# TalShor/SciLMM

Hardware: AMD Instinct MI355X
Metric: REML factorize+solve nnz(L)/s (simulated pedigree, fp64) (higher is better)
Workload: dtype f64

## Files before the change

scilmm_amd/csrc/dev.h:

```cpp
#pragma once
#include <hip/hip_runtime.h>

#include <algorithm>
#include <cstdlib>
#include <optional>
#include <string>
#include <type_traits>
#include <vector>

#include "../../include/scilmm_hip.h"
#include "plan_types.h"
#include "handles.h"

namespace scilmm {

struct Tuning {
  int reserve_cus = 0;
  int side_streams = 2;
  bool no_mfma = false;
  bool trsm_lite = true;
  std::optional<bool> dense;
  std::optional<bool> outside;
  bool outside_merge = true;
  std::optional<int> outside_chunks;
  bool outside_prio = false;
  std::optional<double> cell_limit;
  bool no_lookahead = false;
  int look_depth = 2;
  bool host_cells = false;
  bool no_splitk = false;
  int64_t target_items = 1024;
  int64_t min_item = 24;
  int64_t max_item = 96;
  std::optional<int64_t> dense_items;
  int64_t dense_fill = 256;
  std::optional<bool> dense_taper;
  std::optional<int> dist_group;
  bool dist_nosplit = false;
  int chain_cap = 2048;
  int chain_wide = 12;
  bool no_chain = false;
  int64_t push_slice = 512;
  bool shadow = true;
  int chain_wide_t = 160;
  int chain_full_t = 768;
  bool chain_pipe = true;
  int chain_stagger = 0;
  bool sinv_generic = false;
  bool sinv_reverse = false;
  int sinv_cc_tiles = 2;
};

inline Tuning read_tuning() {
  Tuning t;
  const char* gate = getenv("SCILMM_TUNING");
  if (!(gate && gate[0] == '1')) return t;
  auto env = [](const char* name) { return getenv(name); };
  auto is1 = [&](const char* name) { const char* e = env(name); return e && e[0] == '1'; };
  auto not0 = [&](const char* name) { const char* e = env(name); return !(e && e[0] == '0'); };
  const char* e;
  if ((e = env("SCILMM_RESERVE_CUS"))) t.reserve_cus = atoi(e);
  if ((e = env("SCILMM_SIDE_STREAMS"))) t.side_streams = atoi(e);
  t.no_mfma = is1("SCILMM_NO_MFMA");
  t.trsm_lite = not0("SCILMM_TRSM_LITE");
  if ((e = env("SCILMM_DENSE"))) t.dense = e[0] != '0';
  if ((e = env("SCILMM_OUTSIDE"))) t.outside = e[0] != '0';
  t.outside_merge = not0("SCILMM_OUTSIDE_MERGE");
  if ((e = env("SCILMM_OUTSIDE_CHUNKS"))) t.outside_chunks = atoi(e);
  t.outside_prio = is1("SCILMM_OUTSIDE_PRIO");
  if ((e = env("SCILMM_CELL_LIMIT"))) t.cell_limit = atof(e);
  t.no_lookahead = is1("SCILMM_NO_LOOKAHEAD");
  if ((e = env("SCILMM_LOOK_DEPTH"))) t.look_depth = std::max(1, atoi(e));
  t.host_cells = is1("SCILMM_HOST_CELLS");
  t.no_splitk = is1("SCILMM_NO_SPLITK");
  if ((e = env("SCILMM_TARGET_ITEMS"))) t.target_items = atoll(e);
  if ((e = env("SCILMM_MIN_ITEM"))) t.min_item = atoll(e);
  if ((e = env("SCILMM_MAX_ITEM"))) t.max_item = atoll(e);
  if ((e = env("SCILMM_DENSE_ITEMS"))) t.dense_items = atoll(e);
  if ((e = env("SCILMM_DENSE_FILL"))) t.dense_fill = atoll(e);
  if ((e = env("SCILMM_DENSE_TAPER"))) t.dense_taper = e[0] == '1';
  if ((e = env("SCILMM_DIST_GROUP"))) t.dist_group = atoi(e);
  t.dist_nosplit = is1("SCILMM_DIST_NOSPLIT");
  if ((e = env("SCILMM_CHAIN_CAP"))) t.chain_cap = atoi(e);
  if ((e = env("SCILMM_CHAIN_WIDE"))) t.chain_wide = atoi(e);
  t.no_chain = is1("SCILMM_NO_CHAIN");
  if ((e = env("SCILMM_PUSH_SLICE"))) t.push_slice = atoll(e);
  t.shadow = not0("SCILMM_SHADOW");
  if ((e = env("SCILMM_CHAIN_WIDE_T"))) t.chain_wide_t = atoi(e);
  if ((e = env("SCILMM_CHAIN_FULL_T"))) t.chain_full_t = atoi(e);
  t.chain_pipe = not0("SCILMM_CHAIN_PIPE");
  if ((e = env("SCILMM_CHAIN_STAGGER"))) t.chain_stagger = std::max(0, atoi(e));
  t.sinv_generic = is1("SCILMM_SINV_GENERIC");
  t.sinv_reverse = is1("SCILMM_SINV_REVERSE");
  if ((e = env("SCILMM_SINV_CC_TILES"))) t.sinv_cc_tiles = std::max(1, atoi(e));
  return t;
}

inline bool verbose() { return getenv("SCILMM_VERBOSE") != nullptr; }

struct Dev {
  int device = 0;
  hipStream_t stream = nullptr;
  Tuning tune;
  int prio_lo = 0, prio_hi = 0;
  DevSym v{};
  std::vector<void*> allocs;
  int32_t* d_level_tiles = nullptr;
// ... 293 lines not shown
```

scilmm_amd/csrc/kernels.hip.h:

```cpp
#pragma once
#include <hip/hip_runtime.h>
#ifndef SCILMM_UPD_WAVES
#define SCILMM_UPD_WAVES 2
#endif
#include <stdint.h>
#include <type_traits>

#include "plan_types.h"

namespace scilmm {

typedef double d4 __attribute__((ext_vector_type(4)));

constexpr int NJB = NB / 16;
constexpr int KCS = 16;
constexpr int LDA = TM + 16;
constexpr int LDB = NB + 16;
constexpr int LDP = 34;

__device__ __forceinline__ d4 mfma_f64(double a, double b, d4 c) {
  return __builtin_amdgcn_mfma_f64_16x16x4f64(a, b, c, 0, 0, 0);
}

__global__ void k_assemble(int64_t nnz, const int64_t* __restrict__ dst, ValPtrs vp, double* __restrict__ L) {
// ... 291 lines not shown
  if (wk.slot < 0) {
    double* P = L + S.sn_loff[s];
#pragma unroll
    for (int jb = 0; jb < NJB; ++jb)
#pragma unroll
      for (int r = 0; r < 4; ++r) {
        const int j = 16 * jb + lr + 4 * r;
        const int i = 16 * wv + li;
        if (i < nrow && j < w) P[(int64_t)j * m + R0 + i] -= acc[jb][r];
      }
  } else {
    double* Q = scratch + (int64_t)wk.slot * (TM * NB);
#pragma unroll
    for (int jb = 0; jb < NJB; ++jb)
#pragma unroll
      for (int r = 0; r < 4; ++r) {
        const int j = 16 * jb + lr + 4 * r;
        const int i = 16 * wv + li;
        Q[j * TM + i] = acc[jb][r];
      }
  }
}


#ifndef SCILMM_DENSE_ABL
#define SCILMM_DENSE_ABL 0
#endif
#ifndef SCILMM_DENSE_VEC
#define SCILMM_DENSE_VEC 1
#endif
constexpr int DTR = 2 * TM;
constexpr int KBA = 64;
constexpr int LDA2 = DTR + 16;

#ifdef SCILMM_DENSE_CLK
__device__ unsigned long long g_dense_clk[2];
#endif

__device__ __forceinline__ int64_t uniform_i64(int64_t x) {
  const uint64_t v = (uint64_t)x;
  const uint32_t lo = __builtin_amdgcn_readfirstlane((uint32_t)v), hi = __builtin_amdgcn_readfirstlane((uint32_t)(v >> 32));
  return (int64_t)(((uint64_t)hi << 32) | lo);
}
__device__ __forceinline__ double ld_off(const double* base, uint32_t voff8) {
  return *(const double*)((const char*)base + voff8);
}
__device__ __forceinline__ int uniform_int(int v) { return __builtin_amdgcn_readfirstlane(v); }
typedef __attribute__((address_space(3))) void* lds_vptr;
typedef const __attribute__((address_space(1))) void* gl_vptr;

#ifndef SCILMM_DENSE_B_SG
#define SCILMM_DENSE_B_SG 1
#endif
__global__ __launch_bounds__(512, 1) void k_dense_b(DevSym S, int32_t dense_first, const DenseWork* __restrict__ work,
                                                    double* __restrict__ L, double* __restrict__ scratch,
                                                    const double* __restrict__ zeros) {
  static_assert(NB == 128 && DTR == 256, "k_dense_b: 8 waves x 32 rows, one B k-row per DMA instruction");
  extern __shared__ __attribute__((aligned(16))) double smem[];
  const int tid = threadIdx.x, lane = tid & 63, wv = __builtin_amdgcn_readfirstlane(tid >> 6);
  const int li = lane & 15, lk = lane >> 4;
  const DenseWork wk = work[blockIdx.x];
  const int32_t j = wk.front;
  const int32_t c0j = S.sn_start[j], wj = S.sn_start[j + 1] - c0j;
  const int32_t mj = S.n - c0j;
  const int32_t R0 = wk.ti0 * TM;
  const int32_t nrow = min(wk.ntiles * TM, mj - R0);
  const int32_t ia = 32 * wv + li, ib_ = ia + 16;
  const int32_t ra0 = R0 + (ia < nrow ? ia : 0);
  const int32_t ra1 = R0 + (ib_ < nrow ? ib_ : 0);
  const int32_t b_off = 2 * lane < wj ? 2 * lane : 0;
  const double* zsrc = zeros + 2 * lane;
  struct Chunk { const double* Pd; int32_t md; int kc; uint32_t v0, v1; };
  int32_t kd = wk.k0, kk0 = 0;
  int32_t d_wd = 0, d_md = 0;
  const double* d_P0 = nullptr;
  auto next_chunk = [&]() {
    if (kk0 == 0) {
      const int32_t d = dense_first + kd;
      const int32_t c0d = S.sn_start[d];
      d_wd = __builtin_amdgcn_readfirstlane(S.sn_start[d + 1] - c0d);
      d_md = __builtin_amdgcn_readfirstlane(S.n - c0d);
      d_P0 = L + uniform_i64(S.sn_loff[d] + (c0j - c0d));
    }
    Chunk c;
    c.md = d_md;
    c.Pd = d_P0 + (int64_t)kk0 * d_md;
    c.kc = min(KBA, d_wd - kk0);
    c.v0 = (uint32_t)(lk * c.md + ra0) * 8u;
    c.v1 = (uint32_t)(lk * c.md + ra1) * 8u;
    kk0 += KBA;
    if (kk0 >= d_wd) { kk0 = 0; ++kd; }
    return c;
  };
  auto issue_B = [&](const Chunk& c, int b) {
    double* Bs = smem + b * KBA * LDB;
    if (c.kc == KBA) {
      const double* p = c.Pd + (int64_t)wv * c.md + b_off;
      const int64_t step = 8 * (int64_t)c.md;
#pragma unroll
      for (int i = 0; i < KBA / 8; ++i)
        __builtin_amdgcn_global_load_lds((gl_vptr)(p + i * step), (lds_vptr)(Bs + (wv + 8 * i) * LDB), 16, 0, 0);
      return;
    }
#pragma unroll
    for (int i = 0; i < KBA / 8; ++i) {
      const int kr = wv + 8 * i;
      __builtin_amdgcn_global_load_lds((gl_vptr)(kr < c.kc ? c.Pd + (int64_t)kr * c.md + b_off : zsrc), (lds_vptr)(Bs + kr * LDB), 16, 0, 0);
    }
  };
  auto load_A = [&](const Chunk& c, int s, double (&ra)[4][2]) {
    const int klast = (c.kc - 1) & ~3;
#pragma unroll
    for (int q = 0; q < 4; ++q) {
      const double* sp = c.Pd + (int64_t)min(16 * s + 4 * q, klast) * c.md;
      ra[q][0] = ld_off(sp, c.v0);
      ra[q][1] = ld_off(sp, c.v1);
    }
  };
  d4 acc16[NJB][2];
#pragma unroll
  for (int a = 0; a < NJB; ++a) { acc16[a][0] = (d4){0.0, 0.0, 0.0, 0.0}; acc16[a][1] = (d4){0.0, 0.0, 0.0, 0.0}; }
  if (wk.k0 >= wk.k1) return;
  double rA[2][4][2];
  double bf[2][NJB];
  auto ldB = [&](const double* Bc, int k4, double (&b)[NJB]) {
#pragma unroll
    for (int jb = 0; jb < NJB; ++jb) b[jb] = Bc[(k4 + lk) * LDB + 16 * jb + li];
  };
  auto mma = [&](const double (&b)[NJB], double a0, double a1) {
#pragma unroll
    for (int jb = 0; jb < NJB; ++jb) {
      acc16[jb][0] = mfma_f64(b[jb], a0, acc16[jb][0]);
      acc16[jb][1] = mfma_f64(b[jb], a1, acc16[jb][1]);
    }
  };
  Chunk cur = next_chunk();
  issue_B(cur, 0);
  load_A(cur, 0, rA[0]);
  bool more = kd < wk.k1;
  Chunk nxt = cur;
  if (more) {
    nxt = next_chunk();
    issue_B(nxt, 1);
  }
  asm volatile("s_waitcnt vmcnt(0)" ::: "memory");
  __syncthreads();
  int buf = 0;
  ldB(smem, 0, bf[0]);
  while (true) {
    const double* Bc = smem + buf * KBA * LDB;
    const double* Bn = smem + (buf ^ 1) * KBA * LDB;
    bool more2 = false;
    Chunk nn = nxt;
#pragma unroll
    for (int t = 0; t < 16; ++t) {
      const int s = t >> 2, q = t & 3;
      if (q == 0) {
        if (s < 3) load_A(cur, s + 1, rA[(s + 1) & 1]);
        else if (more) load_A(nxt, 0, rA[0]);
      }
      if (t < 15) {
        ldB(Bc, 4 * (t + 1), bf[(t + 1) & 1]);
      } else if (more) {
        asm volatile("s_waitcnt vmcnt(0) lgkmcnt(0)" ::: "memory");
        __builtin_amdgcn_s_barrier();
        ldB(Bn, 0, bf[0]);
        more2 = kd < wk.k1;
        if (more2) {
          nn = next_chunk();
          issue_B(nn, buf);
        }
      }
      mma(bf[t & 1], rA[s & 1][q][0], rA[s & 1][q][1]);
#if SCILMM_DENSE_B_SG
      if (t < 15) {
#pragma unroll
        for (int g = 0; g < 4; ++g) {
          __builtin_amdgcn_sched_group_barrier(0x100, 1, 0);
          __builtin_amdgcn_sched_group_barrier(0x008, 4, 0);
        }
      }
#endif
      __builtin_amdgcn_sched_barrier(0);
    }
    if (!more) break;
    cur = nxt;
    nxt = nn;
    more = more2;
    buf ^= 1;
  }
  double* P = L + S.sn_loff[j];
#pragma unroll
  for (int jb = 0; jb < NJB; ++jb)
#pragma unroll
    for (int ib = 0; ib < 2; ++ib)
#pragma unroll
      for (int r = 0; r < 4; ++r) {
        const int i = ib == 0 ? ia : ib_, jc = 16 * jb + lk + 4 * r;
        const double v = acc16[jb][ib][r];
        const int h = i >> 7;
        const int32_t slot = h ? wk.slot1 : wk.slot0;
        if (slot < 0) {
          if (i < nrow && jc < wj) P[(int64_t)jc * mj + R0 + i] -= v;
        } else if (h < wk.ntiles) {
          scratch[(int64_t)slot * (TM * NB) + jc * TM + (i & (TM - 1))] = v;
        }
      }
}

typedef float f4 __attribute__((ext_vector_type(4)));
constexpr int LDA2F = DTR + 16;
constexpr int LDBF = NB + 16;

__global__ __launch_bounds__(512, 1) void k_dense32(DevSym S, int32_t dense_first, const DenseWork* __restrict__ work,
                                                    double* __restrict__ L, double* __restrict__ scratch) {
  extern __shared__ __attribute__((aligned(16))) double smem[];
  float* Abuf = (float*)smem;
  float* Bbuf = Abuf + 2 * KC * LDA2F;
  const int tid = threadIdx.x, lane = tid & 63, wv = tid >> 6;
  const DenseWork wk = work[blockIdx.x];
  const int32_t j = wk.front;
  const int32_t c0j = S.sn_start[j], wj = S.sn_start[j + 1] - c0j;
  const int32_t mj = S.n - c0j;
  const int32_t R0 = wk.ti0 * TM;
  const int32_t nrow = min(wk.ntiles * TM, mj - R0);
  typedef double d2 __attribute__((ext_vector_type(2)));
  typedef float f2 __attribute__((ext_vector_type(2)));
  constexpr int NPA = KC / 4, NPB = KC / 8;
  const int pa = tid & (DTR / 2 - 1), ka = tid >> 7;
  const int pb = tid & (NB / 2 - 1), kb = tid >> 6;
  const int ra_row = 2 * pa < nrow ? 2 * pa : 0, rb_col = 2 * pb < wj ? 2 * pb : 0;
  d2 ra[NPA], rb[NPB];
  int32_t kd = wk.k0, kk0 = 0;
  int kc_ld = 0;
  auto load_chunk = [&]() {
    const int32_t d = dense_first + kd;
    const int32_t c0d = S.sn_start[d], wd = S.sn_start[d + 1] - c0d;
    const int64_t md = S.n - c0d;
    const double* Pd = L + S.sn_loff[d] + (int64_t)kk0 * md + (c0j - c0d);
    kc_ld = min(KC, wd - kk0);
#pragma unroll
    for (int i = 0; i < NPA; ++i) __builtin_memcpy(&ra[i], Pd + (int64_t)min(ka + 4 * i, kc_ld - 1) * md + R0 + ra_row, 16);
#pragma unroll
    for (int i = 0; i < NPB; ++i) __builtin_memcpy(&rb[i], Pd + (int64_t)min(kb + 8 * i, kc_ld - 1) * md + rb_col, 16);
    kk0 += KC;
    if (kk0 >= wd) { kk0 = 0; ++kd; }
  };
  auto store_chunk = [&](int b) {
    float* As = Abuf + b * KC * LDA2F;
    float* Bs = Bbuf + b * KC * LDBF;
#pragma unroll
    for (int i = 0; i < NPA; ++i) {
      const bool on = ka + 4 * i < kc_ld;
      *(f2*)&As[(ka + 4 * i) * LDA2F + 2 * pa] = (f2){on ? (float)ra[i][0] : 0.0f, on ? (float)ra[i][1] : 0.0f};
    }
#pragma unroll
    for (int i = 0; i < NPB; ++i) {
      const bool on = kb + 8 * i < kc_ld;
      *(f2*)&Bs[(kb + 8 * i) * LDBF + 2 * pb] = (f2){on ? (float)rb[i][0] : 0.0f, on ? (float)rb[i][1] : 0.0f};
    }
  };
  d4 acc[NJB][2];
#pragma unroll
  for (int a = 0; a < NJB; ++a) { acc[a][0] = (d4){0.0, 0.0, 0.0, 0.0}; acc[a][1] = (d4){0.0, 0.0, 0.0, 0.0}; }
  const int li = lane & 15, lk = lane >> 4;
  if (wk.k0 >= wk.k1) return;
  load_chunk();
  int kc_cur = kc_ld;
  store_chunk(0);
  __syncthreads();
  int buf = 0;
  while (true) {
    const bool more = kd < wk.k1;
    if (more) load_chunk();
    const float* Ac = Abuf + buf * KC * LDA2F;
    const float* Bc = Bbuf + buf * KC * LDBF;
    const int kc4 = (kc_cur + 3) & ~3;
    f4 c32[NJB][2];
#pragma unroll
    for (int a = 0; a < NJB; ++a) { c32[a][0] = (f4){0.f, 0.f, 0.f, 0.f}; c32[a][1] = (f4){0.f, 0.f, 0.f, 0.f}; }
#pragma unroll 2
    for (int k4 = 0; k4 < kc4; k4 += 4) {
      const float a0 = Ac[(k4 + lk) * LDA2F + 32 * wv + li], a1 = Ac[(k4 + lk) * LDA2F + 32 * wv + 16 + li];
      float b[NJB];
#pragma unroll
      for (int jb = 0; jb < NJB; ++jb) b[jb] = Bc[(k4 + lk) * LDBF + 16 * jb + li];
#pragma unroll
      for (int jb = 0; jb < NJB; ++jb) {
        c32[jb][0] = __builtin_amdgcn_mfma_f32_16x16x4f32(b[jb], a0, c32[jb][0], 0, 0, 0);
        c32[jb][1] = __builtin_amdgcn_mfma_f32_16x16x4f32(b[jb], a1, c32[jb][1], 0, 0, 0);
      }
    }
#pragma unroll
    for (int jb = 0; jb < NJB; ++jb)
#pragma unroll
      for (int ib = 0; ib < 2; ++ib)
#pragma unroll
        for (int r = 0; r < 4; ++r) acc[jb][ib][r] += (double)c32[jb][ib][r];
    if (!more) break;
    store_chunk(buf ^ 1);
    kc_cur = kc_ld;
    __syncthreads();
    buf ^= 1;
  }
  double* P = L + S.sn_loff[j];
#pragma unroll
  for (int jb = 0; jb < NJB; ++jb)
#pragma unroll
    for (int ib = 0; ib < 2; ++ib)
#pragma unroll
      for (int r = 0; r < 4; ++r) {
        const int i = 32 * wv + 16 * ib + li, jc = 16 * jb + 4 * lk + r;
        const int h = i >> 7;
        const int32_t slot = h ? wk.slot1 : wk.slot0;
        if (slot < 0) {
          if (i < nrow && jc < wj) P[(int64_t)jc * mj + R0 + i] -= acc[jb][ib][r];
        } else if (h < wk.ntiles) {
          scratch[(int64_t)slot * (TM * NB) + jc * TM + (i & (TM - 1))] = acc[jb][ib][r];
        }
      }
}

__global__ __launch_bounds__(256) void k_shadow(const double* __restrict__ src, float* __restrict__ dst, int64_t cnt) {
  for (int64_t i = (int64_t)blockIdx.x * 256 + threadIdx.x; i < cnt; i += (int64_t)gridDim.x * 256) dst[i] = (float)src[i];
}

#ifndef SCILMM_DENSE_H_FOLD
#define SCILMM_DENSE_H_FOLD 4
#endif
#ifndef SCILMM_DENSE_H_WGS
#define SCILMM_DENSE_H_WGS 4
#endif
constexpr int DH_MAXD = 256;
constexpr size_t dense_h_lds = sizeof(float) * 2 * KBA * LDBF + sizeof(int32_t) * (DH_MAXD + 2) + sizeof(int64_t) * DH_MAXD;

__global__ __launch_bounds__(512, SCILMM_DENSE_H_WGS) void k_dense_h(DevSym S, int32_t dense_first, const DenseWork* __restrict__ work,
                                                    double* __restrict__ L, const float* __restrict__ L32, int64_t base32,
                                                    double* __restrict__ scratch, const float* __restrict__ zeros32) {
  static_assert(NB == 128 && TM == 128, "k_dense_h: 4 x 2 waves of 32 rows x 64 columns");
  extern __shared__ __attribute__((aligned(16))) double smem[];
  float* Bimg = (float*)smem;
  int32_t* t_c0 = (int32_t*)(Bimg + 2 * KBA * LDBF);
  int64_t* t_lo = (int64_t*)(t_c0 + DH_MAXD + 2);
  typedef float f2 __attribute__((ext_vector_type(2)));
  constexpr int NJH = NJB / 2;
  const int tid = threadIdx.x, lane = tid & 63, wv = __builtin_amdgcn_readfirstlane(tid >> 6);
  const int rg = wv >> 1, ch = wv & 1;
  const int li = lane & 15, lk = lane >> 4;
  const DenseWork wk = work[blockIdx.x >> 1];
  const int th = blockIdx.x & 1;
  if (th >= wk.ntiles || wk.k0 >= wk.k1) return;
  const int32_t j = wk.front;
  const int32_t c0j = S.sn_start[j], wj = S.sn_start[j + 1] - c0j;
  const int32_t mj = S.n - c0j;
  const int32_t R0 = (wk.ti0 + th) * TM;
  const int32_t nrow = min(TM, mj - R0);
  const int32_t slot = th ? wk.slot1 : wk.slot0;
  const int32_t ndesc = min(wk.k1 - wk.k0, DH_MAXD);
  for (int i = tid; i <= ndesc; i += 512) t_c0[i] = S.sn_start[dense_first + wk.k0 + i];
  for (int i = tid; i < ndesc; i += 512) t_lo[i] = S.sn_loff[dense_first + wk.k0 + i];
  const int32_t ia = 32 * rg + 2 * li;
  const int32_t ra = R0 + (ia < nrow ? ia : 0);
  const int32_t bcol0 = lane < wj ? lane : 0, bcol1 = 64 + lane < wj ? 64 + lane : 0;
  __syncthreads();
  struct Chunk { const float* Pd; int32_t md; int kc; };
  int32_t kd = wk.k0, kk0 = 0;
  auto next_chunk = [&]() {
    const int32_t e = kd - wk.k0, d = dense_first + kd;
    const bool tab = e < DH_MAXD;
    const int32_t c0d = __builtin_amdgcn_readfirstlane(tab ? t_c0[e] : S.sn_start[d]);
    const int32_t wd = __builtin_amdgcn_readfirstlane(tab ? t_c0[e + 1] : S.sn_start[d + 1]) - c0d;
    Chunk c;
    c.md = S.n - c0d;
    c.Pd = L32 + (uniform_i64(tab ? t_lo[e] : S.sn_loff[d]) - base32 + (int64_t)kk0 * c.md + (c0j - c0d));
    c.kc = min(KBA, wd - kk0);
    kk0 += KBA;
    if (kk0 >= wd) { kk0 = 0; ++kd; }
    return c;
  };
  auto issue_B = [&](const Chunk& c, int b) {
    float* Bs = Bimg + b * KBA * LDBF;
#pragma unroll
    for (int i = 0; i < KBA / 8; ++i) {
      const int kr = wv + 8 * i;
      const float* row = c.Pd + (int64_t)kr * c.md;
      const bool on = kr < c.kc;
      __builtin_amdgcn_global_load_lds((gl_vptr)(on ? row + bcol0 : zeros32 + lane), (lds_vptr)(Bs + kr * LDBF), 4, 0, 0);
      __builtin_amdgcn_global_load_lds((gl_vptr)(on ? row + bcol1 : zeros32 + lane), (lds_vptr)(Bs + kr * LDBF + 64), 4, 0, 0);
    }
  };
  auto load_A = [&](const Chunk& c, int s, f2 (&a)[4]) {
    const int klast = (c.kc - 1) & ~3;
    const uint32_t v = (uint32_t)(lk * c.md + ra) * 4u;
#pragma unroll
    for (int q = 0; q < 4; ++q) {
      const float* sp = c.Pd + (int64_t)min(16 * s + 4 * q, klast) * c.md;
      a[q] = *(const f2*)((const char*)sp + v);
    }
  };
  d4 acc[NJH][2];
  f4 c32[NJH][2];
#pragma unroll
  for (int a = 0; a < NJH; ++a) {
    acc[a][0] = (d4){0.0, 0.0, 0.0, 0.0}; acc[a][1] = (d4){0.0, 0.0, 0.0, 0.0};
// ... 2568 lines not shown
```

scilmm_amd/csrc/launch.hip.h:

```cpp
#pragma once

namespace {

int set_attrs(scilmm_symbolic* sym, Dev* D) {
  if (D->attrs_set) return SCILMM_OK;
  const int big = 150 * 1024;
  HIPCHK(hipFuncSetAttribute((const void*)k_potrf, hipFuncAttributeMaxDynamicSharedMemorySize, big));
  HIPCHK(hipFuncSetAttribute((const void*)k_fwd<true, 0, true>, hipFuncAttributeMaxDynamicSharedMemorySize, big));
  HIPCHK(hipFuncSetAttribute((const void*)k_fwd<true, 0, false>, hipFuncAttributeMaxDynamicSharedMemorySize, big));
  HIPCHK(hipFuncSetAttribute((const void*)k_fwd<true, 1, true>, hipFuncAttributeMaxDynamicSharedMemorySize, big));
  HIPCHK(hipFuncSetAttribute((const void*)k_fwd<false, 0, true>, hipFuncAttributeMaxDynamicSharedMemorySize, big));
  HIPCHK(hipFuncSetAttribute((const void*)k_fwd<false, 0, false>, hipFuncAttributeMaxDynamicSharedMemorySize, big));
  HIPCHK(hipFuncSetAttribute((const void*)k_fwd<false, 1, true>, hipFuncAttributeMaxDynamicSharedMemorySize, big));
  HIPCHK(hipFuncSetAttribute((const void*)k_dense32, hipFuncAttributeMaxDynamicSharedMemorySize, big));
  HIPCHK(hipFuncSetAttribute((const void*)k_dense_h, hipFuncAttributeMaxDynamicSharedMemorySize, big));
  HIPCHK(hipFuncSetAttribute((const void*)k_dense_b, hipFuncAttributeMaxDynamicSharedMemorySize, big));
  HIPCHK(hipFuncSetAttribute((const void*)k_update2<true>, hipFuncAttributeMaxDynamicSharedMemorySize, big));
  HIPCHK(hipFuncSetAttribute((const void*)k_update2<false>, hipFuncAttributeMaxDynamicSharedMemorySize, big));
  D->attrs_set = true;
  return SCILMM_OK;
}

inline int64_t max_groups(unsigned threads) { return (int64_t)(((uint64_t)1 << 32) / threads) - 1; }

struct FactorLaunch {
  Dev* const D;
  scilmm_factor* const fac;
  int64_t launches = 0;

  void update(hipStream_t stream, const UpdWork* work, int64_t cnt, double* scratch_half) {
#ifdef SCILMM_DIAG
    if (D->ablate == 4) return;
#endif
    const size_t sm_upd = sizeof(double) * (size_t)(2 * KC * LDA + 2 * KC * LDB) + sizeof(int32_t) * TM;
    const auto k = D->use_mfma ? k_update2<true> : k_update2<false>;
    for (int64_t o = 0; o < cnt; o += max_groups(UPD_THREADS)) {
      const unsigned c = (unsigned)std::min<int64_t>(cnt - o, max_groups(UPD_THREADS));
      hipLaunchKernelGGL(k, dim3(c), dim3(UPD_THREADS), sm_upd, stream, D->v, work + o, D->d_combos, fac->L, scratch_half);
      launches++;
    }
  }

  void dense(hipStream_t stream, const DenseWork* dw, int64_t cnt, double* scratch_half) {
    const int32_t dense_first = fac->sym->S->dense_first;
    for (int64_t o = 0; o < cnt; o += max_groups(1024)) {
      const unsigned c = (unsigned)std::min<int64_t>(cnt - o, max_groups(1024));
      if (D->front_bits == 32 && fac->L32)
        hipLaunchKernelGGL(k_dense_h, dim3(2 * c), dim3(512), dense_h_lds, stream, D->v, dense_first, dw + o, fac->L, (const float*)fac->L32,
                           fac->base32, scratch_half, (const float*)D->d_zeros);
      else if (D->front_bits == 32)
        hipLaunchKernelGGL(k_dense32, dim3(c), dim3(512), sizeof(float) * (size_t)(2 * KC * LDA2F + 2 * KC * LDBF), stream, D->v,
                           dense_first, dw + o, fac->L, scratch_half);
      else
        hipLaunchKernelGGL(k_dense_b, dim3(c), dim3(512), sizeof(double) * (size_t)(2 * KBA * LDB), stream, D->v, dense_first, dw + o,
                           fac->L, scratch_half, (const double*)D->d_zeros);
      launches++;
    }
  }

  void reduce(hipStream_t stream, const int32_t* tiles, int64_t cnt, const int32_t* pslot, const int32_t* pnseg, const double* slabs) {
    const int64_t per = max_groups(128) / (NB / 4);
    for (int64_t o = 0; o < cnt; o += per) {
      const int64_t c = std::min(cnt - o, per);
      hipLaunchKernelGGL(k_reduce, dim3((unsigned)((NB / 4) * c)), dim3(128), 0, stream, D->v, tiles + o, pslot, pnseg, slabs, fac->L);
      launches++;
    }
  }

  int cells(hipStream_t stream, int which, int32_t l) {
    const Dev::CellSet& CS = D->cellset[which];
    const int64_t u0 = CS.level_ptr[l], u1 = CS.level_ptr[l + 1];
    if (u1 <= u0) return SCILMM_OK;
#ifdef SCILMM_DIAG
    if (D->ablate == 5) return SCILMM_OK;
#endif
    const int64_t nshort = CS.level_short[l], nlong = (u1 - u0) - nshort;
    const int64_t nblk = (nshort + 255) / 256 + (nlong + 3) / 4;
    if (nblk > max_groups(256)) {
      fac->sym->err = "cell plan: one level has more target cells than a dispatch can hold";
      return SCILMM_ERR_ARG;
    }
    hipLaunchKernelGGL(k_sparse_cells, dim3((unsigned)nblk), dim3(256), 0, stream, u0, nshort, u1 - u0, (const int64_t*)CS.dst,
                       (const int64_t*)CS.grp, (const int64_t*)CS.srct, (const int64_t*)CS.srcq, (const int32_t*)CS.md,
                       (const int32_t*)CS.wd, fac->L);
    launches++;
    return SCILMM_OK;
  }

  void trsm(hipStream_t stream, const int32_t* tiles, int64_t cnt, const double* slabs) {
    const bool lite = D->use_mfma && D->trsm_lite;
    const auto k = lite ? k_trsm_lite : D->use_mfma ? k_trsm<true> : k_trsm<false>;
    const int64_t per = lite ? max_groups(256) / 4 : max_groups(256);
    for (int64_t o = 0; o < cnt; o += per) {
      const int64_t c = std::min(cnt - o, per);
      hipLaunchKernelGGL(k, dim3((unsigned)(lite ? 4 * c : c)), dim3(256), 0, stream, D->v, tiles + o, fac->L, fac->invD, D->d_tile_pslot,
                         D->d_tile_pnseg, slabs);
      launches++;
    }
  }

  void outside(hipStream_t stream, const OutsideWork* work, int64_t cnt) {
    auto k = D->use_mfma ? k_outside<true> : k_outside<false>;
#ifdef SCILMM_DIAG
    if (D->ablate == 6) k = k_outside<true, 1>;
    if (D->ablate == 7) k = k_outside<true, 2>;
#endif
    for (int64_t o = 0; o < cnt; o += max_groups(256)) {
      const unsigned c = (unsigned)std::min<int64_t>(max_groups(256), cnt - o);
// ... 112 lines not shown
```

scilmm_amd/csrc/plan.hip:

```cpp
#include <hip/hip_runtime.h>

#include <algorithm>
#include <atomic>
#include <chrono>
#include <functional>
#include <thread>
#include <cmath>
#include <cstdio>
#include <cstdlib>
#include <cstring>
#include <string>
#include <vector>

#include "dev.h"
#include "cellplan.hip.h"
#include "host_threads.h"

namespace scilmm {

void dev_free(void* p) {
  Dev* D = (Dev*)p;
  if (!D) return;
  for (void* a : D->allocs) (void)hipFree(a);
  for (double* v : D->vals)
// ... 942 lines not shown
  int st;
  size_t split = 0;
  int64_t ngroups_total = 0;
  if (pb.gpu_cells) {
    int64_t potential = 0;
    std::vector<const std::vector<CellCombo>*> ccparts;
    for (auto& pv : cellparts) {
      ccparts.push_back(&pv);
      for (const CellCombo& q : pv) potential += (int64_t)q.nt * q.nq;
    }
    if (potential >= ((int64_t)1 << 31)) {
      sym->err = "cell plan: more than 2^31 cells (raise SCILMM_CELL_LIMIT granularity or set SCILMM_HOST_CELLS=1)";
      return SCILMM_ERR_ARG;
    }
    int64_t n_early_groups = 0;
    if ((st = build_cells_device(sym, D, ccparts, std::max(S.nlevels, 1), &ngroups_total, &n_early_groups)) != SCILMM_OK) return st;
    split = (size_t)n_early_groups;
    std::vector<std::vector<CellCombo>>().swap(cellparts);
  } else {
    if ((st = build_cells_host(sym, D, pb, &split, &ngroups_total)) != SCILMM_OK) return st;
  }
  {
    if (pb.verbose)
      fprintf(stderr, "[scilmm plan] dense combos %lld, cell-path combos %lld, cells %lld (early %lld) in %lld target groups\n",
              (long long)D->n_dense_combos, (long long)D->n_sparse_combos, (long long)D->n_cells, (long long)split,
              (long long)ngroups_total);
    std::vector<Cell>().swap(cells);
  }
  return SCILMM_OK;
}

struct WorkCut {
  const Symbolic& S;
  Dev* const D;
  const PlanBuild& pb;
  const std::vector<int64_t>&dptr, &dmid;
  std::vector<int32_t> pslot, pnseg, pslot_e, pnseg_e, red_tiles, red_tiles_e;
  std::vector<UpdWork> work, work_early;
  std::vector<DenseWork> dwork_e, dwork_l;
  int64_t max_slots = 0;
  const bool lookahead = !D->tune.no_lookahead;
  const int32_t depth = D->look_depth;
  const bool allow_split = !D->tune.no_splitk;
  const int64_t target_items = D->tune.target_items, min_item = D->tune.min_item, max_item = std::max<int64_t>(min_item, D->tune.max_item);
  const int64_t dense_fill = D->tune.dense_fill;
  const int32_t tail_w = tail_width(S);
  const int64_t dense_items = std::max<int64_t>(64, D->tune.dense_items.value_or(tail_w < 24576 ? 128 : tail_w < 32768 ? 512 : 1024));
  std::vector<std::vector<int32_t>> tail_src;
  std::vector<int32_t> tail_col_front;
  const bool dist = distributed_tail(D, S);
  const int32_t Wg = D->dist_Wg;
  std::vector<std::vector<uint8_t>> own_pair_on;
  int64_t dense_pairs_all = 0, dense_pairs_kept = 0, dense_tiles_all = 0, dense_tiles_kept = 0;

  WorkCut(const Symbolic& S_, Dev* D_, const PlanBuild& pb_) : S(S_), D(D_), pb(pb_), dptr(pb_.dptr), dmid(pb_.dmid) {
    const int64_t ntiles = (int64_t)S.tile_front.size();
    pslot.assign((size_t)std::max<int64_t>(ntiles, 1), 0);
    pnseg.assign(pslot.size(), 0);
    pslot_e.assign(pslot.size(), 0);
    pnseg_e.assign(pslot.size(), 0);
    D->red_ptr_e.assign(S.nlevels + 1, 0);
    D->dwork_e_ptr.assign(S.nlevels + 1, 0);
    D->dwork_l_ptr.assign(S.nlevels + 1, 0);
    D->dwork_l_mid.assign((size_t)std::max(S.nlevels, 1), 0);
    D->work_ptr.assign(S.nlevels + 1, 0);
    D->early_ptr.assign(S.nlevels + 1, 0);
    D->red_ptr.assign(S.nlevels + 1, 0);
    if (D->dense_on && !S.tail_blk_ptr.empty()) {
      const int32_t nT = S.nsuper - S.dense_first;
      tail_src.resize((size_t)nT);
      for (int32_t d = 0; d < nT; ++d)
        for (int64_t e = S.tail_blk_ptr[d]; e < S.tail_blk_ptr[d + 1]; ++e) tail_src[(size_t)S.tail_blk[e]].push_back(d);
    }
    if (!tail_src.empty()) {
      const int32_t c0t = S.sn_start[S.dense_first];
      tail_col_front.resize((size_t)(S.n - c0t));
      for (int32_t f = S.dense_first; f < S.nsuper; ++f)
        for (int32_t c = S.sn_start[f]; c < S.sn_start[f + 1]; ++c) tail_col_front[(size_t)(c - c0t)] = f - S.dense_first;
    }
    if (dist) own_pair_on.resize((size_t)(S.nsuper - S.dense_first));
  }

  int64_t combo_cost(int64_t c) const { return pb.cd_cost[(size_t)c]; }
  int64_t cut(int32_t g, int64_t cb, int64_t ce, int64_t per_item, std::vector<UpdWork>& out) const {
    if (ce <= cb) return 0;
    int64_t tcost = 0;
    for (int64_t c = cb; c < ce; ++c) tcost += combo_cost(c);
    const int64_t nseg = std::min<int64_t>(64, std::max<int64_t>(1, (tcost + per_item / 2) / per_item));
    const int64_t seg_cost = (tcost + nseg - 1) / nseg;
    const size_t first = out.size();
    int64_t a = cb, acc = 0;
    for (int64_t c = cb; c < ce; ++c) {
      acc += combo_cost(c);
      if (nseg > 1 && acc >= seg_cost && c + 1 < ce) {
        out.push_back(UpdWork{g, 0, a, c + 1});
        a = c + 1;
        acc = 0;
      }
    }
    out.push_back(UpdWork{g, 0, a, ce});
    return (int64_t)(out.size() - first);
  }
  int64_t active_runs(int32_t jj, int32_t lo, int32_t hi, std::vector<std::pair<int32_t, int32_t>>& runs) const {
    runs.clear();
    if (hi <= lo) return 0;
    if (tail_src.empty()) {
// ... 165 lines not shown
    for (size_t oi = 0; oi < order.size(); ++oi) {
      const int32_t g = order[oi];
      const size_t fe = work_early.size(), fl = work.size();
      const int64_t ne = cut(g, dptr[g], dmid[g], per_e, work_early);
      const int64_t nl = cut(g, dmid[g], dptr[g + 1], per_l, work);
      const bool dtile = dj >= 0 && S.tile_front[g] == dj && pair_on[(size_t)((g - S.tile_base[dj]) / 2)];
      const int64_t dte = dtile ? nde : 0, dtl = dtile ? ndl : 0;
      const int64_t pe = (ne + dte) >= 2 ? ne : 0, pl = (nl + dtl) >= 2 ? nl : 0;
      const int64_t pde = (ne + dte) >= 2 ? dte : 0, pdl = (nl + dtl) >= 2 ? dtl : 0;
      if (ne == 1 && pe == 0) work_early[fe].slot = -1;
      if (nl == 1 && pl == 0) work[fl].slot = -1;
      if (pe + pde > 0) {
        pslot_e[g] = (int32_t)slots;
        pnseg_e[g] = (int32_t)(pe + pde);
        red_tiles_e.push_back(g);
        for (int64_t k = 0; k < pe; ++k) work_early[fe + k].slot = (int32_t)(slots + k);
        if (pde > 0) dbase_e[(size_t)(g - S.tile_base[dj])] = (int32_t)(slots + pe);
        slots += pe + pde;
      }
      if (pl + pdl > 0) {
        pslot[g] = (int32_t)slots;
        pnseg[g] = (int32_t)(pl + pdl);
        red_tiles.push_back(g);
        for (int64_t k = 0; k < pl; ++k) work[fl + k].slot = (int32_t)(slots + k);
        if (pdl > 0) dbase_l[(size_t)(g - S.tile_base[dj])] = (int32_t)(slots + pl);
        slots += pl + pdl;
      }
    }
    {
      auto seg_major = [&](std::vector<UpdWork>& v, size_t first) {
        if (v.size() - first < 2) return;
        std::vector<std::pair<int32_t, int32_t>> key(v.size() - first);
        int32_t seg = 0;
        for (size_t k = first; k < v.size(); ++k) {
          seg = (k > first && v[k].tile == v[k - 1].tile) ? seg + 1 : 0;
          key[k - first] = {seg, (int32_t)(k - first)};
        }
        std::stable_sort(key.begin(), key.end(), [](const std::pair<int32_t, int32_t>& a, const std::pair<int32_t, int32_t>& b) { return a.first < b.first; });
        std::vector<UpdWork> tmp(v.begin() + first, v.end());
        for (size_t k = 0; k < key.size(); ++k) v[first + k] = tmp[(size_t)key[k].second];
      };
      seg_major(work_early, (size_t)D->early_ptr[l]);
      seg_major(work, (size_t)D->work_ptr[l]);
    }
    return slots;
  }

  void emit_dense_items(const DenseLevel& dl, const std::vector<int32_t>& dbase_e, const std::vector<int32_t>& dbase_l) {
    const int32_t dj = dl.dj;
    const std::vector<uint8_t>& pair_on = dl.pair_on;
    const std::vector<std::pair<int32_t, int32_t>>&segs_e = dl.segs_e, &segs_l = dl.segs_l;
    if (dj >= 0) {
      const int32_t ntl = (int32_t)(S.tile_base[dj + 1] - S.tile_base[dj]);
      auto emit = [&](std::vector<DenseWork>& out, const std::vector<std::pair<int32_t, int32_t>>& segs, const std::vector<int32_t>& base) {
        for (size_t sg = 0; sg < segs.size(); ++sg) {
          const int32_t k0 = segs[sg].first, k1 = segs[sg].second;
          for (int32_t q = 0; q < ntl; q += 2) {
            if (!pair_on[(size_t)(q / 2)]) continue;
            const int32_t nt2 = std::min<int32_t>(2, ntl - q);
            DenseWork wk{dj, q, nt2, k0, k1, base[(size_t)q] < 0 ? -1 : base[(size_t)q] + (int32_t)sg,
                         (nt2 == 2 && base[(size_t)q + 1] >= 0) ? base[(size_t)q + 1] + (int32_t)sg : -1, 0};
            out.push_back(wk);
          }
        }
      };
      emit(dwork_e, segs_e, dbase_e);
      emit(dwork_l, segs_l, dbase_l);
    }
  }

  void cut_level(int32_t l) {
    int64_t total_e = 0, total_l = 0;
    for (int64_t i = S.level_tile_ptr[l]; i < S.level_tile_ptr[l + 1]; ++i) {
      const int32_t g = S.level_tiles[i];
      for (int64_t c = dptr[g]; c < dmid[g]; ++c) total_e += combo_cost(c);
      for (int64_t c = dmid[g]; c < dptr[g + 1]; ++c) total_l += combo_cost(c);
    }
    const DenseLevel dl = plan_dense_level(l);
    total_e += dl.cost_e;
    total_l += dl.cost_l;
    std::vector<int32_t> dbase_e, dbase_l;
    const int64_t slots = cut_explicit_items(l, dl, total_e, total_l, dbase_e, dbase_l);
    emit_dense_items(dl, dbase_e, dbase_l);
    const int32_t dj = dl.dj, nseg_older = dl.nseg_older;
    const std::vector<uint8_t>& pair_on = dl.pair_on;
    D->dwork_e_ptr[l + 1] = (int64_t)dwork_e.size();
    D->dwork_l_ptr[l + 1] = (int64_t)dwork_l.size();
    {
      int64_t np_on_l = 0;
      if (dj >= 0 && nseg_older >= 0)
        for (uint8_t v : pair_on) np_on_l += v;
      D->dwork_l_mid[(size_t)l] = (dj >= 0 && nseg_older >= 0) ? D->dwork_l_ptr[l] + (int64_t)nseg_older * np_on_l : D->dwork_l_ptr[l + 1];
    }
    max_slots = std::max(max_slots, slots);
    D->lev_cost_e.push_back(total_e);
    D->lev_cost_l.push_back(total_l);
    D->work_ptr[l + 1] = (int64_t)work.size();
    D->early_ptr[l + 1] = (int64_t)work_early.size();
    D->red_ptr[l + 1] = (int64_t)red_tiles.size();
    D->red_ptr_e[l + 1] = (int64_t)red_tiles_e.size();
  }

  int plan_dist_batches(scilmm_symbolic* sym) {
    int st;
    const int32_t nT = S.nsuper - S.dense_first;
    const int32_t ngroups = (nT + Wg - 1) / Wg;
    std::vector<DenseWork> dwork_b;
    D->dbatch_ptr.assign((size_t)ngroups + 1, 0);
    std::vector<std::pair<int32_t, int32_t>> runs;
    for (int32_t g = 0; g < ngroups; ++g) {
      for (int32_t jj = (g + 2) * Wg; jj < nT; ++jj) {
        const int32_t fr = S.dense_first + jj;
        if (!D->keep_front[fr]) continue;
        if (active_runs(jj, g * Wg, std::min((g + 1) * Wg, nT), runs) == 0) continue;
        const int32_t k0 = runs.front().first, k1 = runs.back().second;
        const int32_t ntl = (int32_t)(S.tile_base[fr + 1] - S.tile_base[fr]);
        const std::vector<uint8_t>& pon = own_pair_on[(size_t)jj];
        for (int32_t q = 0; q < ntl; q += 2) {
          if (!pon.empty() && !pon[(size_t)(q / 2)]) continue;
          dwork_b.push_back(DenseWork{fr, q, std::min<int32_t>(2, ntl - q), k0, k1, -1, -1, 0});
        }
      }
      D->dbatch_ptr[(size_t)g + 1] = (int64_t)dwork_b.size();
    }
    if (dwork_b.empty()) dwork_b.push_back(DenseWork{});
    if ((st = upload(sym, D, dwork_b, &D->d_dwork_b)) != SCILMM_OK) return st;
    if (pb.verbose)
      fprintf(stderr, "[scilmm plan] rank %d: %lld batch items in %d source groups of %d tail panels\n", D->rank,
              (long long)D->dbatch_ptr[(size_t)ngroups], ngroups, Wg);
    return SCILMM_OK;
  }

  void report_slabs(const char* cls, int64_t items, const std::vector<int32_t>& tiles, const std::vector<int32_t>& nseg) const {
    int64_t slabs = 0, odd = 0;
    int32_t lo = 0, hi = 0;
    for (int32_t g : tiles) {
      const int32_t c = nseg[(size_t)g];
      slabs += c;
      odd += c & 1;
      lo = lo == 0 ? c : std::min(lo, c);
      hi = std::max(hi, c);
    }
    fprintf(stderr, "[scilmm plan] %s: %lld explicit items, %lld partial slabs on %zu tiles, %d .. %d per tile, %lld tiles with an odd count, %lld with an even one\n",
            cls, (long long)items, (long long)slabs, tiles.size(), lo, hi, (long long)odd, (long long)((int64_t)tiles.size() - odd));
  }

  int upload_items(scilmm_symbolic* sym) {
    int st;
    if (pb.verbose) {
      report_slabs("early launches", (int64_t)work_early.size(), red_tiles_e, pnseg_e);
      report_slabs("late launches", (int64_t)work.size(), red_tiles, pnseg);
      fprintf(stderr, "[scilmm plan] split-K %s, panel solve %s, %d side streams\n", allow_split ? "on" : "off",
              !D->use_mfma ? "k_trsm<false>" : D->trsm_lite ? "k_trsm_lite" : "k_trsm<true>", D->nside);
    }
    {
      if (dwork_e.empty()) dwork_e.push_back(DenseWork{});
      if (dwork_l.empty()) dwork_l.push_back(DenseWork{});
      if ((st = upload(sym, D, dwork_e, &D->d_dwork_e)) != SCILMM_OK) return st;
      if ((st = upload(sym, D, dwork_l, &D->d_dwork_l)) != SCILMM_OK) return st;
      if (pb.verbose && dense_pairs_all > 0)
        fprintf(stderr, "[scilmm plan] dense tail: %lld of %lld (target, descendant) panel pairs carry true entries, %lld of %lld target tile pairs are reached by a descendant (the others are padding only and skipped)\n",
                (long long)dense_pairs_kept, (long long)dense_pairs_all, (long long)dense_tiles_kept, (long long)dense_tiles_all);
      if (pb.verbose)
        fprintf(stderr, "[scilmm plan] dense tail: fronts %d..%d (%d wide), %lld early + %lld late implicit items (k_dense_b)\n",
                S.dense_first, S.nsuper - 1, tail_w,
                (long long)D->dwork_e_ptr[S.nlevels], (long long)D->dwork_l_ptr[S.nlevels]);
    }
    if (work_early.empty()) work_early.push_back(UpdWork{0, -1, 0, 0});
    if ((st = upload(sym, D, work_early, &D->d_work_early)) != SCILMM_OK) return st;
    if (red_tiles_e.empty()) red_tiles_e.push_back(0);
    if ((st = upload(sym, D, red_tiles_e, &D->d_red_tiles_e)) != SCILMM_OK) return st;
    if ((st = upload(sym, D, pslot_e, &D->d_tile_pslot_e)) != SCILMM_OK) return st;
    if ((st = upload(sym, D, pnseg_e, &D->d_tile_pnseg_e)) != SCILMM_OK) return st;
    if (red_tiles.empty()) red_tiles.push_back(0);
    if ((st = upload(sym, D, red_tiles, &D->d_red_tiles)) != SCILMM_OK) return st;
    if (work.empty()) work.push_back(UpdWork{0, -1, 0, 0});
    if ((st = upload(sym, D, work, &D->d_work)) != SCILMM_OK) return st;
    if ((st = upload(sym, D, pslot, &D->d_tile_pslot)) != SCILMM_OK) return st;
    if ((st = upload(sym, D, pnseg, &D->d_tile_pnseg)) != SCILMM_OK) return st;
    void* sc = nullptr;
    HIPCHK(hipMalloc(&sc, sizeof(double) * (size_t)4 * (size_t)D->max_slots * TM * NB));
    D->allocs.push_back(sc);
    D->scratch = (double*)sc;
    return SCILMM_OK;
  }
};

int cut_work_items(scilmm_symbolic* sym, Dev* D, PlanBuild& pb) {
  WorkCut wc(*sym->S, D, pb);
  for (int32_t l = 0; l < sym->S->nlevels; ++l) wc.cut_level(l);
  D->max_slots = std::max<int64_t>(wc.max_slots, 1);
  int st;
  if (wc.dist && (st = wc.plan_dist_batches(sym)) != SCILMM_OK) return st;
  return wc.upload_items(sym);
}

int plan_chain(scilmm_symbolic* sym, Dev* D, PlanBuild& pb) {
  const Symbolic& S = *sym->S;
  int st;
  const int32_t ns = S.nsuper;
  const int32_t cap = D->tune.chain_cap, wide = D->tune.chain_wide;
  int32_t l0 = S.nlevels;
  while (l0 > 0 && S.level_ptr[l0] - S.level_ptr[l0 - 1] <= wide && S.level_ptr[S.nlevels] - S.level_ptr[l0 - 1] <= cap) --l0;
  int32_t T = l0 < S.nlevels ? S.level_ptr[S.nlevels] - S.level_ptr[l0] : 0;
  if (S.nlevels - l0 < 4 || D->tune.no_chain) T = 0;
  if (D->world > 1) T = 0;
  D->chain_T = T;
  D->chain_l0 = l0;
  if (T > 0 && D->det) {
    std::vector<uint8_t> mask((size_t)ns, 0);
    for (int32_t i = 0; i < T; ++i) mask[(size_t)S.level_fronts[S.level_ptr[l0] + i]] = 1;
    if ((st = upload(sym, D, mask, &D->d_chain_mask)) != SCILMM_OK) return st;
  }
  if (T > 0) {
    std::vector<int32_t> chain(T), pos(ns, -1);
// ... 382 lines not shown
```

Before: 1.437 billion.

## Pipeline dense-tail descriptor and A loads, and trim per-pair descendant ranges

```diff
diff --git a/scilmm_amd/csrc/dev.h b/scilmm_amd/csrc/dev.h
--- a/scilmm_amd/csrc/dev.h
+++ b/scilmm_amd/csrc/dev.h
@@ -42,6 +42,7 @@
   bool no_chain = false;
   int64_t push_slice = 512;
   bool shadow = true;
+  bool dense_feed = true;
   int chain_wide_t = 160;
   int chain_full_t = 768;
   bool chain_pipe = true;
@@ -51,8 +52,15 @@
   int sinv_cc_tiles = 2;
 };
 
+inline bool read_dense_feed() {
+  const char* gate = getenv("SCILMM_TUNING");
+  const char* e = getenv("SCILMM_DENSE_FEED");
+  return !(gate && gate[0] == '1' && e && e[0] == '0');
+}
+
 inline Tuning read_tuning() {
   Tuning t;
+  t.dense_feed = read_dense_feed();
   const char* gate = getenv("SCILMM_TUNING");
   if (!(gate && gate[0] == '1')) return t;
   auto env = [](const char* name) { return getenv(name); };
diff --git a/scilmm_amd/csrc/kernels.hip.h b/scilmm_amd/csrc/kernels.hip.h
--- a/scilmm_amd/csrc/kernels.hip.h
+++ b/scilmm_amd/csrc/kernels.hip.h
@@ -367,6 +367,24 @@
 #ifndef SCILMM_DENSE_B_SG
 #define SCILMM_DENSE_B_SG 1
 #endif
+__device__ __forceinline__ void dense_empty_item(const DenseWork& wk, double* __restrict__ scratch, int tile) {
+  for (int h = 0; h < wk.ntiles; ++h) {
+    const int32_t slot = h ? wk.slot1 : wk.slot0;
+    if (slot < 0 || (tile >= 0 && tile != h)) continue;
+    double* sl = scratch + (int64_t)slot * (TM * NB);
+    for (int i = threadIdx.x; i < TM * NB; i += blockDim.x) sl[i] = 0.0;
+  }
+}
+#define SCILMM_WAIT_A(a, N)                                                                                                \
+  asm volatile("s_waitcnt vmcnt(" #N ")"                                                                                   \
+               : "+v"(a[0][0]), "+v"(a[0][1]), "+v"(a[1][0]), "+v"(a[1][1]), "+v"(a[2][0]), "+v"(a[2][1]), "+v"(a[3][0]), "+v"(a[3][1]))
+#define SCILMM_WAIT_A2(a, flag, N1, N0)                                                                                    \
+  asm volatile("s_cmp_eq_u32 %8, 0\n\ts_cbranch_scc1 .Lwa0_%=\n\ts_waitcnt vmcnt(" #N1 ")\n\ts_branch .Lwa1_%=\n"            \
+               ".Lwa0_%=:\n\ts_waitcnt vmcnt(" #N0 ")\n.Lwa1_%=:"                                                          \
+               : "+v"(a[0][0]), "+v"(a[0][1]), "+v"(a[1][0]), "+v"(a[1][1]), "+v"(a[2][0]), "+v"(a[2][1]), "+v"(a[3][0]), "+v"(a[3][1])  \
+               : "s"(uniform_int((int)(flag)))                                                                                       \
+               : "scc")
+template <int FEED>
 __global__ __launch_bounds__(512, 1) void k_dense_b(DevSym S, int32_t dense_first, const DenseWork* __restrict__ work,
                                                     double* __restrict__ L, double* __restrict__ scratch,
                                                     const double* __restrict__ zeros) {
@@ -389,8 +407,25 @@
   int32_t kd = wk.k0, kk0 = 0;
   int32_t d_wd = 0, d_md = 0;
   const double* d_P0 = nullptr;
+  int32_t n_wd = 0, n_md = 0;
+  const double* n_P0 = nullptr;
+  auto fetch_desc = [&]() {
+    const int32_t d = uniform_int(dense_first + kd);
+    uint64_t c01;
+    int64_t lo;
+    asm volatile("s_load_dwordx2 %0, %2, 0x0\n\ts_load_dwordx2 %1, %3, 0x0\n\ts_waitcnt lgkmcnt(0)"
+                 : "=&s"(c01), "=&s"(lo)
+                 : "s"(S.sn_start + d), "s"(S.sn_loff + d)
+                 : "memory");
+    const int32_t c0d = (int32_t)(uint32_t)c01;
+    n_wd = (int32_t)(uint32_t)(c01 >> 32) - c0d;
+    n_md = S.n - c0d;
+    n_P0 = L + (lo + (c0j - c0d));
+  };
   auto next_chunk = [&]() {
-    if (kk0 == 0) {
+    if (FEED == 2) {
+      if (kk0 == 0) { d_wd = n_wd; d_md = n_md; d_P0 = n_P0; }
+    } else if (kk0 == 0) {
       const int32_t d = dense_first + kd;
       const int32_t c0d = S.sn_start[d];
       d_wd = __builtin_amdgcn_readfirstlane(S.sn_start[d + 1] - c0d);
@@ -428,14 +463,19 @@
 #pragma unroll
     for (int q = 0; q < 4; ++q) {
       const double* sp = c.Pd + (int64_t)min(16 * s + 4 * q, klast) * c.md;
-      ra[q][0] = ld_off(sp, c.v0);
-      ra[q][1] = ld_off(sp, c.v1);
+      if (FEED == 2) {
+        asm volatile("global_load_dwordx2 %0, %1, %2" : "=v"(ra[q][0]) : "v"(c.v0), "s"(sp));
+        asm volatile("global_load_dwordx2 %0, %1, %2" : "=v"(ra[q][1]) : "v"(c.v1), "s"(sp));
+      } else {
+        ra[q][0] = ld_off(sp, c.v0);
+        ra[q][1] = ld_off(sp, c.v1);
+      }
     }
   };
   d4 acc16[NJB][2];
 #pragma unroll
   for (int a = 0; a < NJB; ++a) { acc16[a][0] = (d4){0.0, 0.0, 0.0, 0.0}; acc16[a][1] = (d4){0.0, 0.0, 0.0, 0.0}; }
-  if (wk.k0 >= wk.k1) return;
+  if (wk.k0 >= wk.k1) { dense_empty_item(wk, scratch, -1); return; }
   double rA[2][4][2];
   double bf[2][NJB];
   auto ldB = [&](const double* Bc, int k4, double (&b)[NJB]) {
@@ -449,19 +489,26 @@
       acc16[jb][1] = mfma_f64(b[jb], a1, acc16[jb][1]);
     }
   };
+  if (FEED == 2) fetch_desc();
   Chunk cur = next_chunk();
   issue_B(cur, 0);
   load_A(cur, 0, rA[0]);
   bool more = kd < wk.k1;
   Chunk nxt = cur;
   if (more) {
+    if (FEED == 2 && kk0 == 0) fetch_desc();
     nxt = next_chunk();
     issue_B(nxt, 1);
   }
   asm volatile("s_waitcnt vmcnt(0)" ::: "memory");
+  if (FEED == 2) SCILMM_WAIT_A(rA[0], 0);
   __syncthreads();
   int buf = 0;
   ldB(smem, 0, bf[0]);
+#ifdef SCILMM_DENSE_CLK
+  uint64_t clk_wait = 0;
+  const uint64_t clk_0 = __builtin_amdgcn_s_memtime();
+#endif
   while (true) {
     const double* Bc = smem + buf * KBA * LDB;
     const double* Bn = smem + (buf ^ 1) * KBA * LDB;
@@ -473,12 +520,25 @@
       if (q == 0) {
         if (s < 3) load_A(cur, s + 1, rA[(s + 1) & 1]);
         else if (more) load_A(nxt, 0, rA[0]);
+        if (FEED == 2) {
+          if (s == 0) SCILMM_WAIT_A2(rA[0], more, 16, 8);
+          else if (s < 3) SCILMM_WAIT_A(rA[s & 1], 8);
+          else SCILMM_WAIT_A2(rA[1], more, 8, 0);
+          if (s == 2 && more && kk0 == 0 && kd < wk.k1) fetch_desc();
+        }
       }
       if (t < 15) {
         ldB(Bc, 4 * (t + 1), bf[(t + 1) & 1]);
       } else if (more) {
-        asm volatile("s_waitcnt vmcnt(0) lgkmcnt(0)" ::: "memory");
+#ifdef SCILMM_DENSE_CLK
+        const uint64_t clk_b = __builtin_amdgcn_s_memtime();
+#endif
+        if (FEED != 0) asm volatile("s_waitcnt vmcnt(8) lgkmcnt(0)" ::: "memory");
+        else asm volatile("s_waitcnt vmcnt(0) lgkmcnt(0)" ::: "memory");
         __builtin_amdgcn_s_barrier();
+#ifdef SCILMM_DENSE_CLK
+        clk_wait += __builtin_amdgcn_s_memtime() - clk_b;
+#endif
         ldB(Bn, 0, bf[0]);
         more2 = kd < wk.k1;
         if (more2) {
@@ -504,6 +564,12 @@
     more = more2;
     buf ^= 1;
   }
+#ifdef SCILMM_DENSE_CLK
+  if (tid == 0) {
+    atomicAdd(&g_dense_clk[0], (unsigned long long)(__builtin_amdgcn_s_memtime() - clk_0));
+    atomicAdd(&g_dense_clk[1], (unsigned long long)clk_wait);
+  }
+#endif
   double* P = L + S.sn_loff[j];
 #pragma unroll
   for (int jb = 0; jb < NJB; ++jb)
@@ -579,7 +645,7 @@
 #pragma unroll
   for (int a = 0; a < NJB; ++a) { acc[a][0] = (d4){0.0, 0.0, 0.0, 0.0}; acc[a][1] = (d4){0.0, 0.0, 0.0, 0.0}; }
   const int li = lane & 15, lk = lane >> 4;
-  if (wk.k0 >= wk.k1) return;
+  if (wk.k0 >= wk.k1) { dense_empty_item(wk, scratch, -1); return; }
   load_chunk();
   int kc_cur = kc_ld;
   store_chunk(0);
@@ -664,7 +730,8 @@
   const int li = lane & 15, lk = lane >> 4;
   const DenseWork wk = work[blockIdx.x >> 1];
   const int th = blockIdx.x & 1;
-  if (th >= wk.ntiles || wk.k0 >= wk.k1) return;
+  if (th >= wk.ntiles) return;
+  if (wk.k0 >= wk.k1) { dense_empty_item(wk, scratch, th); return; }
   const int32_t j = wk.front;
   const int32_t c0j = S.sn_start[j], wj = S.sn_start[j + 1] - c0j;
   const int32_t mj = S.n - c0j;
diff --git a/scilmm_amd/csrc/launch.hip.h b/scilmm_amd/csrc/launch.hip.h
--- a/scilmm_amd/csrc/launch.hip.h
+++ b/scilmm_amd/csrc/launch.hip.h
@@ -14,7 +14,8 @@
   HIPCHK(hipFuncSetAttribute((const void*)k_fwd<false, 1, true>, hipFuncAttributeMaxDynamicSharedMemorySize, big));
   HIPCHK(hipFuncSetAttribute((const void*)k_dense32, hipFuncAttributeMaxDynamicSharedMemorySize, big));
   HIPCHK(hipFuncSetAttribute((const void*)k_dense_h, hipFuncAttributeMaxDynamicSharedMemorySize, big));
-  HIPCHK(hipFuncSetAttribute((const void*)k_dense_b, hipFuncAttributeMaxDynamicSharedMemorySize, big));
+  HIPCHK(hipFuncSetAttribute((const void*)k_dense_b<2>, hipFuncAttributeMaxDynamicSharedMemorySize, big));
+  HIPCHK(hipFuncSetAttribute((const void*)k_dense_b<0>, hipFuncAttributeMaxDynamicSharedMemorySize, big));
   HIPCHK(hipFuncSetAttribute((const void*)k_update2<true>, hipFuncAttributeMaxDynamicSharedMemorySize, big));
   HIPCHK(hipFuncSetAttribute((const void*)k_update2<false>, hipFuncAttributeMaxDynamicSharedMemorySize, big));
   D->attrs_set = true;
@@ -27,6 +28,7 @@
   Dev* const D;
   scilmm_factor* const fac;
   int64_t launches = 0;
+  const bool dense_feed = read_dense_feed();
 
   void update(hipStream_t stream, const UpdWork* work, int64_t cnt, double* scratch_half) {
 #ifdef SCILMM_DIAG
@@ -52,8 +54,9 @@
         hipLaunchKernelGGL(k_dense32, dim3(c), dim3(512), sizeof(float) * (size_t)(2 * KC * LDA2F + 2 * KC * LDBF), stream, D->v,
                            dense_first, dw + o, fac->L, scratch_half);
       else
-        hipLaunchKernelGGL(k_dense_b, dim3(c), dim3(512), sizeof(double) * (size_t)(2 * KBA * LDB), stream, D->v, dense_first, dw + o,
-                           fac->L, scratch_half, (const double*)D->d_zeros);
+        hipLaunchKernelGGL(dense_feed ? k_dense_b<2> : k_dense_b<0>, dim3(c), dim3(512),
+                           sizeof(double) * (size_t)(2 * KBA * LDB), stream, D->v, dense_first, dw + o, fac->L, scratch_half,
+                           (const double*)D->d_zeros);
       launches++;
     }
   }
diff --git a/scilmm_amd/csrc/plan.hip b/scilmm_amd/csrc/plan.hip
--- a/scilmm_amd/csrc/plan.hip
+++ b/scilmm_amd/csrc/plan.hip
@@ -1018,6 +1018,7 @@
   const int32_t Wg = D->dist_Wg;
   std::vector<std::vector<uint8_t>> own_pair_on;
   int64_t dense_pairs_all = 0, dense_pairs_kept = 0, dense_tiles_all = 0, dense_tiles_kept = 0;
+  int64_t dense_prod_all = 0, dense_prod_kept = 0, dense_items_empty = 0;
 
   WorkCut(const Symbolic& S_, Dev* D_, const PlanBuild& pb_) : S(S_), D(D_), pb(pb_), dptr(pb_.dptr), dmid(pb_.dmid) {
     const int64_t ntiles = (int64_t)S.tile_front.size();
@@ -1289,11 +1290,35 @@
     const std::vector<std::pair<int32_t, int32_t>>&segs_e = dl.segs_e, &segs_l = dl.segs_l;
     if (dj >= 0) {
       const int32_t ntl = (int32_t)(S.tile_base[dj + 1] - S.tile_base[dj]);
+      const int32_t jj = dj - S.dense_first;
+      const bool reach_known = !tail_src.empty() && jj > 0;
+      const int32_t c0t = S.sn_start[S.dense_first], c0j = S.sn_start[dj];
+      auto trim = [&](int32_t q, int32_t& k0, int32_t& k1) {
+        if (!reach_known || k1 <= k0) return;
+        const int64_t lo = (int64_t)c0j + (int64_t)TM * q, hi = std::min<int64_t>(lo + 2 * TM, S.n);
+        const int32_t f_lo = tail_col_front[(size_t)(lo - c0t)], f_hi = tail_col_front[(size_t)(hi - 1 - c0t)];
+        if (f_lo <= jj) return;
+        int32_t first = k1, last = k0 - 1;
+        for (int32_t f = f_lo; f <= f_hi; ++f) {
+          const std::vector<int32_t>& sf = tail_src[(size_t)f];
+          const auto a = std::lower_bound(sf.begin(), sf.end(), k0), b = std::lower_bound(sf.begin(), sf.end(), k1);
+          if (a != b) {
+            first = std::min(first, *a);
+            last = std::max(last, *(b - 1));
+          }
+        }
+        if (first > last) k1 = k0;
+        else { k0 = first; k1 = last + 1; }
+      };
       auto emit = [&](std::vector<DenseWork>& out, const std::vector<std::pair<int32_t, int32_t>>& segs, const std::vector<int32_t>& base) {
         for (size_t sg = 0; sg < segs.size(); ++sg) {
-          const int32_t k0 = segs[sg].first, k1 = segs[sg].second;
           for (int32_t q = 0; q < ntl; q += 2) {
             if (!pair_on[(size_t)(q / 2)]) continue;
+            int32_t k0 = segs[sg].first, k1 = segs[sg].second;
+            dense_prod_all += k1 - k0;
+            trim(q, k0, k1);
+            dense_prod_kept += k1 - k0;
+            dense_items_empty += k1 <= k0 ? 1 : 0;
             const int32_t nt2 = std::min<int32_t>(2, ntl - q);
             DenseWork wk{dj, q, nt2, k0, k1, base[(size_t)q] < 0 ? -1 : base[(size_t)q] + (int32_t)sg,
                          (nt2 == 2 && base[(size_t)q + 1] >= 0) ? base[(size_t)q + 1] + (int32_t)sg : -1, 0};
@@ -1398,6 +1423,9 @@
       if (pb.verbose && dense_pairs_all > 0)
         fprintf(stderr, "[scilmm plan] dense tail: %lld of %lld (target, descendant) panel pairs carry true entries, %lld of %lld target tile pairs are reached by a descendant (the others are padding only and skipped)\n",
                 (long long)dense_pairs_kept, (long long)dense_pairs_all, (long long)dense_tiles_kept, (long long)dense_tiles_all);
+      if (pb.verbose && dense_prod_all > 0)
+        fprintf(stderr, "[scilmm plan] dense tail: per-pair reach keeps %lld of %lld (tile pair, descendant) products, %lld empty items (zero slabs)\n",
+                (long long)dense_prod_kept, (long long)dense_prod_all, (long long)dense_items_empty);
       if (pb.verbose)
         fprintf(stderr, "[scilmm plan] dense tail: fronts %d..%d (%d wide), %lld early + %lld late implicit items (k_dense_b)\n",
                 S.dense_first, S.nsuper - 1, tail_w,
```

Result: faster. 1.483 billion (median of 6 runs) (+3.2%).
